# fusioninfer/fusioninfer

Hardware: AMD Instinct MI355X
Metric: goodput req/s (Qwen3-8B serving, closed-loop) (higher is better)
Workload: dtype bf16; 1 GPU; model=Qwen3-8B, global_batch=256, seq_len=1152, prompt_len=1024, gen_len=128, parallelism=dp1

## Files before the change

### fusioninfer_amd/engine/model_runner.py

```python

from __future__ import annotations

import os
from typing import Dict, List, Optional, Tuple

import numpy as np
import torch

from fusioninfer_amd.config import EngineConfig
from fusioninfer_amd.engine.block_manager import BlockManager
from fusioninfer_amd.engine.metadata import AttnMetadata
from fusioninfer_amd.engine.sequence import Sequence
from fusioninfer_amd.models.model import CausalLM
import fusioninfer_amd.ops as ops_mod

_DECODE_BUCKETS = [1, 2, 4, 8, 16, 24, 32, 48, 64, 96, 128, 160, 192, 224, 256, 320, 384, 448, 512]


class ModelRunner:
    def __init__(self, cfg: EngineConfig, device: str):
        self.cfg = cfg
        self.device = torch.device(device)
        self.is_cuda = self.device.type == "cuda"
        mc = cfg.model
# ... 149 lines not shown
            "lora_names": [s.lora_name for s in seqs],
        }

    def _lora_route(self, prefill_payload, decode_payload, np_=0):
        if self.lora_registry is None:
            return None
        spans: List[Tuple[int, int, str]] = []
        total = 0
        if prefill_payload is not None:
            cu = prefill_payload["cu"]
            total = cu[-1]
            for i, name in enumerate(prefill_payload.get("lora_names") or []):
                if name:
                    spans.append((cu[i], cu[i + 1], name))
        if decode_payload is not None:
            total = np_ + len(decode_payload["lens"])
            for i, name in enumerate(decode_payload.get("lora_names") or []):
                if name:
                    spans.append((np_ + i, np_ + i + 1, name))
        if not spans:
            return None
        reg = self.lora_registry
        adapters = {}
        for _, _, name in spans:
            if name not in adapters:
                adapters[name] = reg.get(name)
        if self.lora_slots is not None and len(adapters) <= reg.max_loras:
            slot = {name: reg.slot_of(name) for name in adapters}
            if all(s is not None for s in slot.values()):
                ids = np.full(total, -1, dtype=np.int32)
                for a, b, name in spans:
                    ids[a:b] = slot[name]
                self.num_lora_slot_steps += 1
                return "slots", ids
        groups: Dict[str, List[int]] = {}
        for a, b, name in spans:
            groups.setdefault(name, []).extend(range(a, b))
        self.num_lora_loop_steps += 1
        return "loop", [(adapters[n], rows) for n, rows in groups.items()]

    def _lora_batch(self, prefill_payload, decode_payload, np_=0):
        route = self._lora_route(prefill_payload, decode_payload, np_)
        if route is None:
            return None
        from fusioninfer_amd.lora import LoRABatch

        kind, data = route
        if kind == "slots":
            return LoRABatch(
                slot_ids=torch.from_numpy(data).to(self.device),
                slots=self.lora_slots,
            )
        return self._lora_batch_from_groups(data)

    def _lora_batch_from_groups(self, groups):
        from fusioninfer_amd.lora import LoRABatch

        return LoRABatch(
            [
                (
                    adapter,
                    torch.tensor(rows, dtype=torch.long, device=self.device),
                )
                for adapter, rows in groups
            ]
        )

    def run_prefill(self, payload) -> torch.Tensor:
        import fusioninfer_amd.distributed.parallel_state as ps

        if ps.pp_world_size() > 1:
            subs = self._split_prefill_payload(payload)
            if len(subs) > 1:
                return self._run_prefill_pp_pipelined(subs)
        ids, meta, logits_idx = self._prefill_inputs(payload)
        with torch.no_grad():
            return self._forward_and_logits(ids, meta, logits_idx)

    def _prefill_inputs(self, payload):
        dev = self.device
        cu = payload["cu"]
        tile_rows = ops_mod.prefill_tile_rows(payload["new_lens"])
        tile_seq, tile_row0 = ops_mod.build_prefill_tiles(
            payload["new_lens"], device=dev, rows=tile_rows
        )
        meta = AttnMetadata(
            num_prefill_tokens=cu[-1],
            num_decode_tokens=0,
            positions=torch.tensor(
                payload["positions"], dtype=torch.int32, device=dev
            ),
            slot_mapping=torch.tensor(
                payload["slots"], dtype=torch.int32, device=dev
            ),
            cu_seqlens=torch.tensor(cu, dtype=torch.int32, device=dev),
            tile_seq=tile_seq,
            tile_rows=tile_rows,
            tile_row0=tile_row0,
            prefill_block_tables=torch.tensor(
                payload["bt"], dtype=torch.int32, device=dev
            ),
            prefill_seq_lens_k=torch.tensor(
                payload["total_lens"], dtype=torch.int32, device=dev
            ),
        )
        meta.lora = self._lora_batch(payload, None)
        ids = torch.tensor(payload["ids"], dtype=torch.long, device=dev)
        if payload.get("logits_rows") is not None:
            logits_idx = torch.tensor(
                payload["logits_rows"], dtype=torch.long, device=dev
            )
        else:
            sample = payload.get("sample") or [True] * (len(cu) - 1)
            logits_idx = torch.tensor(
                [c - 1 for c, smp in zip(cu[1:], sample) if smp],
                dtype=torch.long,
                device=dev,
            )
        return ids, meta, logits_idx

    def _split_prefill_payload(self, payload, min_mb_tokens: int = 256):
        import fusioninfer_amd.distributed.parallel_state as ps

        cu = payload["cu"]
        n_seqs = len(cu) - 1
        M = min(ps.pp_world_size(), n_seqs, cu[-1] // min_mb_tokens)
        if M < 2:
            return [payload]
        target = cu[-1] / M
        bounds = [0]
        for i in range(1, M):
            want = i * target
            j = bounds[-1] + 1
            while j < n_seqs - (M - 1 - i) and cu[j + 1] <= want:
                j += 1
            bounds.append(j)
        bounds.append(n_seqs)
        rows = payload.get("logits_rows")
        subs = []
        for a, b in zip(bounds, bounds[1:]):
            lo, hi = cu[a], cu[b]
            sp = {
                "kind": "prefill",
                "ids": payload["ids"][lo:hi],
                "positions": payload["positions"][lo:hi],
                "slots": payload["slots"][lo:hi],
                "cu": [c - lo for c in cu[a: b + 1]],
                "new_lens": payload["new_lens"][a:b],
                "total_lens": payload["total_lens"][a:b],
                "bt": payload["bt"][a:b],
                "sample": payload["sample"][a:b],
                "lora_names": (payload.get("lora_names") or [None] * n_seqs)[a:b],
            }
            if rows is not None:
                sp["logits_rows"] = [r - lo for r in rows if lo <= r < hi]
            subs.append(sp)
        return subs

    def _run_prefill_pp_pipelined(self, subs) -> torch.Tensor:
        import fusioninfer_amd.distributed.parallel_state as ps

        V = self.cfg.model.vocab_size
        H = self.cfg.model.hidden_size
        dt = torch.bfloat16
        dev = self.device
        last = ps.pp_world_size() - 1
        inputs = [self._prefill_inputs(sp) for sp in subs]
# ... 112 lines not shown
        payload["kind"] = "mixed"
        d = (
            self.build_decode_payload(decode_seqs, bm)
            if decode_seqs
            else {"ids": [], "positions": [], "slots": [], "lens": [], "bt": []}
        )
        payload["decode"] = d
        return payload

    def build_spec_payload(
        self,
        prefill_seqs: List[Sequence],
        chunks: List[int],
        decode_seqs: List[Sequence],
        drafts: List[List[int]],
        bm: BlockManager,
    ):
        input_ids: List[int] = []
        positions: List[int] = []
        slots: List[int] = []
        cu = [0]
        new_lens: List[int] = []
        total_lens: List[int] = []
        sample: List[bool] = []
        logits_rows: List[int] = []
        bs = bm.block_size
        all_seqs = list(prefill_seqs) + list(decode_seqs)

        def _extend(seq, toks, C):
            chunk = len(toks)
            input_ids.extend(toks)
            positions.extend(range(C, C + chunk))
            pos = np.arange(C, C + chunk)
            blocks = np.asarray(seq.block_ids, dtype=np.int64)
            slots.extend((blocks[pos // bs] * bs + pos % bs).tolist())
            cu.append(cu[-1] + chunk)
            new_lens.append(chunk)
            total_lens.append(C + chunk)

        for seq, chunk in zip(prefill_seqs, chunks):
            C = seq.num_computed_tokens or seq.num_cached_tokens
            _extend(seq, seq.all_token_ids[C: C + chunk], C)
            done = C + chunk >= seq.num_prompt_tokens
            sample.append(done)
            if done:
                logits_rows.append(cu[-1] - 1)
        for seq, draft in zip(decode_seqs, drafts):
            row0 = cu[-1]
            _extend(seq, [seq.all_token_ids[-1]] + list(draft),
                    seq.num_tokens - 1)
            sample.append(True)
            logits_rows.extend(range(row0, cu[-1]))
        max_blocks = max(len(s.block_ids) for s in all_seqs)
        bt = [
            s.block_ids + [0] * (max_blocks - len(s.block_ids))
            for s in all_seqs
        ]
        return {
            "kind": "prefill",
            "ids": input_ids,
            "positions": positions,
            "slots": slots,
            "cu": cu,
            "new_lens": new_lens,
            "total_lens": total_lens,
            "bt": bt,
            "sample": sample,
            "logits_rows": logits_rows,
            "lora_names": [s.lora_name for s in all_seqs],
        }

    def run_batch(self, payload) -> torch.Tensor:
        d = payload["decode"]
        if not payload["ids"]:
            return self.run_decode(d)
        if not d["ids"]:
            return self.run_prefill(payload)
        dev = self.device
        cu = payload["cu"]
        np_ = cu[-1]
        nd = len(d["ids"])
        tile_rows = ops_mod.prefill_tile_rows(payload["new_lens"])
        tile_seq, tile_row0 = ops_mod.build_prefill_tiles(
            payload["new_lens"], device=dev, rows=tile_rows
        )
        max_blocks = max(len(b) for b in d["bt"])
        dbt_np = np.zeros((nd, max_blocks), dtype=np.int32)
        for i, ids in enumerate(d["bt"]):
            dbt_np[i, : len(ids)] = ids
        dbt = torch.from_numpy(dbt_np)
        meta = AttnMetadata(
            num_prefill_tokens=np_,
            num_decode_tokens=nd,
            positions=torch.tensor(
                payload["positions"] + d["positions"],
                dtype=torch.int32, device=dev,
            ),
            slot_mapping=torch.tensor(
                payload["slots"] + d["slots"], dtype=torch.int32, device=dev
            ),
            cu_seqlens=torch.tensor(cu, dtype=torch.int32, device=dev),
            tile_seq=tile_seq,
            tile_rows=tile_rows,
            tile_row0=tile_row0,
            prefill_block_tables=torch.tensor(
                payload["bt"], dtype=torch.int32, device=dev
            ),
            prefill_seq_lens_k=torch.tensor(
                payload["total_lens"], dtype=torch.int32, device=dev
            ),
            block_tables=dbt.to(dev),
            seq_lens=torch.tensor(d["lens"], dtype=torch.int32, device=dev),
        )
        meta.lora = self._lora_batch(payload, d, np_=np_)
        ids = torch.tensor(
            payload["ids"] + d["ids"], dtype=torch.long, device=dev
        )
        if payload.get("logits_rows") is not None:
            logits_idx = torch.tensor(
                payload["logits_rows"], dtype=torch.long, device=dev
            )
        else:
            pf_idx = [
                c - 1 for c, smp in zip(cu[1:], payload["sample"]) if smp
            ]
            logits_idx = torch.tensor(
                pf_idx + list(range(np_, np_ + nd)), dtype=torch.long,
                device=dev,
            )
        with torch.no_grad():
            return self._forward_and_logits(ids, meta, logits_idx)

    def _alloc_static(self, max_bs: int) -> None:
        dev = self.device
        self._static = {
            "ids": torch.zeros(max_bs, dtype=torch.long, device=dev),
            "positions": torch.zeros(max_bs, dtype=torch.int32, device=dev),
            "slots": torch.full((max_bs,), -1, dtype=torch.int32, device=dev),
            "block_tables": torch.zeros(
                (max_bs, self.max_blocks_per_seq), dtype=torch.int32, device=dev
            ),
            "seq_lens": torch.ones(max_bs, dtype=torch.int32, device=dev),
        }
        if self.lora_slots is not None:
            self._static["lora_slots"] = torch.full(
                (max_bs,), -1, dtype=torch.int32, device=dev
            )

    def _decode_forward(self, bs: int, lora=None) -> torch.Tensor:
        s = self._static
        meta = AttnMetadata(
            num_prefill_tokens=0,
            num_decode_tokens=bs,
            lora=lora,
            positions=s["positions"][:bs],
            slot_mapping=s["slots"][:bs],
            block_tables=s["block_tables"][:bs],
            seq_lens=s["seq_lens"][:bs],
        )
        return self._forward_and_logits(
            s["ids"][:bs], meta,
            torch.arange(bs, dtype=torch.long, device=self.device),
        )

    def capture_decode_graphs(self) -> None:
        import fusioninfer_amd.distributed.parallel_state as ps

# ... 139 lines not shown
```

### fusioninfer_amd/ops/__init__.py

```python

from __future__ import annotations

import math
from typing import Optional

import torch

from fusioninfer_amd.ops import reference as ref

_C = None
_C_IMPORT_ERROR: Optional[BaseException] = None
try:
    import importlib

    _C = importlib.import_module("fusioninfer_amd.ops._C")
except Exception as e:
    _C_IMPORT_ERROR = e


def has_native() -> bool:
    return _C is not None


def _require_native():
# ... 170 lines not shown
        _require_native()
        n = int(block_ids.numel())
        staging = torch.empty(
            (2, n, *k_cache.shape[1:]), dtype=k_cache.dtype, device=k_cache.device
        )
        _C.gather_kv_blocks(staging, k_cache, v_cache, block_ids)
        return staging
    return ref.gather_kv_blocks(k_cache, v_cache, block_ids.long())


def scatter_kv_blocks(staging, k_cache, v_cache, block_ids):
    if k_cache.is_cuda:
        _require_native()
        _C.scatter_kv_blocks(staging, k_cache, v_cache, block_ids)
        return
    ref.scatter_kv_blocks(staging, k_cache, v_cache, block_ids.long())



DECODE_PARTITION_TOKENS = 512


def _check_attn_out(out: torch.Tensor, q: torch.Tensor) -> None:
    if (out.shape != q.shape or out.dtype != q.dtype
            or out.device != q.device or not out.is_contiguous()):
        raise ValueError(
            f"out must be a contiguous {tuple(q.shape)} {q.dtype} tensor on "
            f"{q.device}, got {tuple(out.shape)} {out.dtype} strides "
            f"{out.stride()} on {out.device}")


def paged_attention_decode(
    q: torch.Tensor,
    k_cache: torch.Tensor,
    v_cache: torch.Tensor,
    block_tables: torch.Tensor,
    seq_lens: torch.Tensor,
    scale: Optional[float] = None,
    out: Optional[torch.Tensor] = None,
) -> torch.Tensor:
    if scale is None:
        scale = 1.0 / math.sqrt(q.shape[-1])
    if out is not None:
        _check_attn_out(out, q)
    if q.is_cuda:
        _require_native()
        S, Hq, D = q.shape
        if out is None:
            out = torch.empty(q.shape, dtype=q.dtype, device=q.device)
        max_tokens = int(block_tables.shape[1]) * int(k_cache.shape[2])
        num_parts = max(
            (max_tokens + DECODE_PARTITION_TOKENS - 1) // DECODE_PARTITION_TOKENS,
            1,
        )
        ml_ws = acc_ws = None
        if num_parts > 1:
            ml_ws = torch.empty(
                (S, Hq, num_parts, 2), dtype=torch.float32, device=q.device
            )
            acc_ws = torch.empty(
                (S, Hq, num_parts, D), dtype=torch.float32, device=q.device
            )
        _C.paged_attention_decode(
            out, q, k_cache, v_cache, block_tables, seq_lens,
            ml_ws, acc_ws, num_parts, scale,
        )
        return out
    res = ref.paged_attention_decode(q, k_cache, v_cache, block_tables, seq_lens, scale)
    return res if out is None else out.copy_(res)


import os as _os

PREFILL_TILE_ROWS = (4 if _os.environ.get("FI_PF_NW", "8").startswith("4")
                     else 8) * 32


def prefill_tile_rows(seq_lens) -> int:
    if seq_lens and max(seq_lens) >= 4096:
        return 128
    return PREFILL_TILE_ROWS


def build_prefill_tiles(seq_lens, device=None, rows=None):
    rows = rows or PREFILL_TILE_ROWS
    tile_seq, tile_row0 = [], []
    for s, L in enumerate(seq_lens):
        for r0 in range(0, L, rows):
            tile_seq.append(s)
            tile_row0.append(r0)
    return (
        torch.tensor(tile_seq, dtype=torch.int32, device=device),
        torch.tensor(tile_row0, dtype=torch.int32, device=device),
    )


def prefill_attention(
    q: torch.Tensor,
    k: torch.Tensor,
    v: torch.Tensor,
    cu_seqlens: torch.Tensor,
    scale: Optional[float] = None,
    tile_seq: Optional[torch.Tensor] = None,
    tile_row0: Optional[torch.Tensor] = None,
    tile_rows: Optional[int] = None,
) -> torch.Tensor:
    if scale is None:
        scale = 1.0 / math.sqrt(q.shape[-1])
    if q.is_cuda:
        _require_native()
        if tile_seq is None:
            lens = (cu_seqlens[1:] - cu_seqlens[:-1]).tolist()
            tile_rows = tile_rows or prefill_tile_rows(lens)
            tile_seq, tile_row0 = build_prefill_tiles(
                lens, device=q.device, rows=tile_rows
            )
        out = torch.empty(q.shape, dtype=q.dtype, device=q.device)
        _C.prefill_attention(out, q, k, v, tile_seq, tile_row0, cu_seqlens,
                             scale, tile_rows or PREFILL_TILE_ROWS)
        return out
    return ref.prefill_attention(q, k, v, cu_seqlens, scale, causal=True)


def prefill_attention_paged(
    q: torch.Tensor,
    k_cache: torch.Tensor,
    v_cache: torch.Tensor,
    block_tables: torch.Tensor,
    cu_seqlens_q: torch.Tensor,
    seq_lens_k: torch.Tensor,
    scale: Optional[float] = None,
    tile_seq: Optional[torch.Tensor] = None,
    tile_row0: Optional[torch.Tensor] = None,
    tile_rows: Optional[int] = None,
    out: Optional[torch.Tensor] = None,
) -> torch.Tensor:
    if scale is None:
        scale = 1.0 / math.sqrt(q.shape[-1])
    if out is not None:
        _check_attn_out(out, q)
    if q.is_cuda:
        _require_native()
        if tile_seq is None:
            lens = (cu_seqlens_q[1:] - cu_seqlens_q[:-1]).tolist()
            tile_rows = tile_rows or prefill_tile_rows(lens)
            tile_seq, tile_row0 = build_prefill_tiles(
                lens, device=q.device, rows=tile_rows
            )
        if out is None:
            out = torch.empty(q.shape, dtype=q.dtype, device=q.device)
        _C.prefill_attention_paged(
            out, q, k_cache, v_cache, tile_seq, tile_row0, cu_seqlens_q,
            block_tables, seq_lens_k, scale,
            tile_rows or PREFILL_TILE_ROWS,
        )
        return out
    res = ref.prefill_attention_paged(
        q, k_cache, v_cache, block_tables, cu_seqlens_q, seq_lens_k, scale
    )
    return res if out is None else out.copy_(res)



def pack_moe_weights(w: torch.Tensor) -> torch.Tensor:
    E, K, N = w.shape
    assert K % 32 == 0 and N % 16 == 0, (K, N)
    return (
        w.view(E, K // 32, 4, 8, N // 16, 16)
        .permute(0, 1, 4, 2, 5, 3)
        .reshape(E, K // 32, N // 16, 64, 8)
        .contiguous()
    )


def moe_gemm(out, a, b_packed, sorted_ids, expert_ids, n_valid,
             block_m: int, gate_up: bool):
    if out.is_cuda:
        _require_native()
        _C.moe_gemm(out, a, b_packed, sorted_ids, expert_ids, n_valid,
                    block_m, gate_up)
        return out
    return ref.moe_gemm(out, a, b_packed, sorted_ids, expert_ids, n_valid,
                        block_m, gate_up)


def moe_gemm_fp8(out, a, a_scales, b_packed, b_scales, sorted_ids,
                 expert_ids, n_valid, block_m: int, gate_up: bool):
    if out.is_cuda:
        _require_native()
        _C.moe_gemm_fp8(out, a, a_scales, b_packed, b_scales, sorted_ids,
                        expert_ids, n_valid, block_m, gate_up)
        return out
    return ref.moe_gemm_fp8(out, a, a_scales, b_packed, b_scales,
                            sorted_ids, expert_ids, n_valid, block_m,
                            gate_up)


def moe_align(topi: torch.Tensor, e_start: int, e_end: int, block_m: int):
    _require_native()
    T, k = topi.shape
    n = T * k
    E_local = e_end - e_start
    PM = ((n + block_m - 1) // block_m + E_local) * block_m
    dev = topi.device
    sorted_ids = torch.empty(PM, dtype=torch.int32, device=dev)
    expert_ids = torch.empty(PM // block_m, dtype=torch.int32, device=dev)
    n_valid = torch.empty(1, dtype=torch.int32, device=dev)
    pos = torch.empty(n, dtype=torch.int32, device=dev)
    _C.moe_align(topi.reshape(-1).int().contiguous(), sorted_ids,
                 expert_ids, n_valid, pos, k, e_start, e_end, block_m)
    return sorted_ids, expert_ids, n_valid, pos, PM


def moe_router_topk(logits: torch.Tensor, k: int, renorm: bool):
    _require_native()
    T, E = logits.shape
    topv = torch.empty(T, k, dtype=torch.float32, device=logits.device)
    topi = torch.empty(T, k, dtype=torch.int32, device=logits.device)
    _C.moe_router_topk(logits.contiguous(), topv, topi, k, renorm)
    return topv, topi


def moe_combine(out, y, pos, w):
    if out.is_cuda:
        _require_native()
        _C.moe_combine(out, y, pos, w)
        return out
    return ref.moe_combine(out, y, pos, w)



LORA_MAX_RANK = 128


def lora_shapes_supported(K: int, N: int, R: int) -> bool:
    return (K % 64 == 0 and N % 16 == 0 and R % 16 == 0
            and 16 <= R <= LORA_MAX_RANK)
# ... 217 lines not shown
```

### fusioninfer_amd/ops/csrc/ops.hip

```cpp

#include <torch/extension.h>

#include <c10/hip/HIPStream.h>
#include <hip/hip_runtime.h>

#include "common.h"

namespace fi {

template <bool FUSED_ADD, bool FP8_OUT>
void launch_rms_norm(void*, float*, const u16*, u16*, const u16*, float, int,
                     int, hipStream_t);
void launch_silu_and_mul(u16*, const u16*, int64_t, int, hipStream_t);
template <bool SILU_MUL>
void launch_row_quant_fp8(unsigned char*, float*, const u16*, int, int,
                          hipStream_t);
void launch_rope_qk_norm(u16*, u16*, int64_t, int64_t, const u16*, const u16*,
                         const float*, const int*, int, int, int, int, float,
                         hipStream_t);
void launch_reshape_and_cache(const u16*, const u16*, void*, void*,
                              const int*, int64_t, int64_t, int, int, int,
                              int, bool, float, float, hipStream_t);
void launch_rope_qk_norm_cache(u16*, const u16*, const u16*, int64_t, int64_t,
                               int64_t, const u16*, const u16*, const float*,
                               const int*, void*, void*, const int*, int, int,
                               int, int, float, bool, float, float,
                               hipStream_t);
template <bool GATHER>
void launch_kv_block_copy(u16*, u16*, u16*, const int*, int, int64_t,
                          hipStream_t);
void launch_paged_attn_decode(u16*, float*, float*, const u16*, const void*,
                              const void*, const int*, const int*, int,
                              int64_t, int, int, int, int, int, float, bool,
                              hipStream_t);
void launch_prefill_attn(u16*, const u16*, const void*, const void*,
                         const int*, const int*, const int*, const int*,
                         const int*, int, int, int64_t, int64_t, int64_t, int,
                         int, int, float, bool, int, hipStream_t);
void launch_moe_gemm(u16*, const u16*, const u16*, const int*, const int*,
                     const int*, int, int, int, int, bool, hipStream_t);
void launch_moe_gemm_fp8(u16*, const unsigned char*, const float*,
                         const unsigned char*, const float*, const int*,
                         const int*, const int*, int, int, int, int, bool,
                         hipStream_t);
void launch_moe_align(const int*, int*, int*, int*, int*, int, int, int,
                      int, int, int, hipStream_t);
void launch_moe_router_topk(const float*, float*, int*, int, int, int,
                            bool, hipStream_t);
void launch_moe_combine(u16*, const u16*, const int*, const float*, int, int,
                        int, hipStream_t);
void launch_lora_apply(u16*, u16*, const u16*, const int*, const u16*,
                       const u16*, const float*, int, int, int, int, int,
                       hipStream_t);
void launch_sample_tokens(int64_t*, const float*, const float*, const int*,
                          const float*, const float*, const int64_t*, int,
                          int, hipStream_t);
void launch_token_logprobs(float*, int*, float*, const float*, const int64_t*,
                           const int*, int, int, int, hipStream_t);
void launch_apply_penalties(float*, const int*, const int*, const float*, int,
                            int, int, hipStream_t);
void launch_penalty_counts_add(int*, const int*, const int64_t*, int, int,
                               int, hipStream_t);

}

namespace {

using fi::u16;

#define CHECK_BF16_CUDA(t)                                     \
  TORCH_CHECK((t).is_cuda(), #t " must be on GPU");            \
  TORCH_CHECK((t).scalar_type() == at::kBFloat16, #t " must be bf16")

u16* bf16_ptr(at::Tensor& t) { return reinterpret_cast<u16*>(t.data_ptr()); }
const u16* bf16_cptr(const at::Tensor& t) {
  return reinterpret_cast<const u16*>(t.data_ptr());
}

hipStream_t current_stream() {
  return c10::hip::getCurrentHIPStream().stream();
}

bool cache_is_fp8(const at::Tensor& t) {
  TORCH_CHECK(
      t.scalar_type() == at::kBFloat16 || t.scalar_type() == at::kFloat8_e4m3fn,
      "kv cache must be bf16 or float8_e4m3fn");
  return t.scalar_type() == at::kFloat8_e4m3fn;
}

void rms_norm(at::Tensor out, at::Tensor input, at::Tensor weight, double eps) {
  CHECK_BF16_CUDA(out);
  CHECK_BF16_CUDA(input);
  TORCH_CHECK(input.is_contiguous() && out.is_contiguous());
  const int hidden = input.size(-1);
  const int tokens = input.numel() / hidden;
  fi::launch_rms_norm<false, false>(bf16_ptr(out), nullptr, bf16_cptr(input),
                                    nullptr, bf16_cptr(weight),
                                    static_cast<float>(eps), tokens, hidden,
                                    current_stream());
}

void fused_add_rms_norm(at::Tensor input, at::Tensor residual,
                        at::Tensor weight, double eps) {
  CHECK_BF16_CUDA(input);
  CHECK_BF16_CUDA(residual);
  TORCH_CHECK(input.is_contiguous() && residual.is_contiguous());
  const int hidden = input.size(-1);
  const int tokens = input.numel() / hidden;
  fi::launch_rms_norm<true, false>(bf16_ptr(input), nullptr, bf16_cptr(input),
                                   bf16_ptr(residual), bf16_cptr(weight),
                                   static_cast<float>(eps), tokens, hidden,
                                   current_stream());
}

#define CHECK_FP8_OUT(o, s)                                                  \
  TORCH_CHECK((o).scalar_type() == at::kFloat8_e4m3fn && (o).is_cuda() &&    \
              (o).is_contiguous());                                          \
  TORCH_CHECK((s).scalar_type() == at::kFloat && (s).is_cuda())

void rms_norm_fp8(at::Tensor out, at::Tensor out_scales, at::Tensor input,
                  at::Tensor weight, double eps) {
// ... 156 lines not shown
  const u16* qw = weight_ptr(q_weight);
  const u16* kw = weight_ptr(k_weight);
  fi::launch_rope_qk_norm_cache(
      bf16_ptr(q), bf16_cptr(k), bf16_cptr(v), q.stride(0), k.stride(0),
      v.stride(0), qw, kw, cos_sin.data_ptr<float>(),
      positions.data_ptr<int>(), k_cache.data_ptr(), v_cache.data_ptr(),
      slot_mapping.data_ptr<int>(), static_cast<int>(tokens),
      static_cast<int>(num_q_heads), static_cast<int>(num_kv_heads),
      static_cast<int>(head_dim), static_cast<float>(eps), fp8,
      static_cast<float>(k_inv_scale), static_cast<float>(v_inv_scale),
      current_stream());
}

void gather_kv_blocks(at::Tensor staging, at::Tensor k_cache,
                      at::Tensor v_cache, at::Tensor block_ids) {
  TORCH_CHECK(staging.is_cuda() &&
              staging.scalar_type() == k_cache.scalar_type());
  TORCH_CHECK(block_ids.scalar_type() == at::kInt);
  const int n = block_ids.size(0);
  const int64_t block_elems = k_cache.size(1) * k_cache.size(2) *
      k_cache.size(3) * k_cache.element_size() / 2;
  fi::launch_kv_block_copy<true>(
      static_cast<fi::u16*>(staging.data_ptr()),
      static_cast<fi::u16*>(k_cache.data_ptr()),
      static_cast<fi::u16*>(v_cache.data_ptr()), block_ids.data_ptr<int>(), n,
      block_elems, current_stream());
}

void scatter_kv_blocks(at::Tensor staging, at::Tensor k_cache,
                       at::Tensor v_cache, at::Tensor block_ids) {
  TORCH_CHECK(staging.is_cuda() &&
              staging.scalar_type() == k_cache.scalar_type());
  TORCH_CHECK(block_ids.scalar_type() == at::kInt);
  const int n = block_ids.size(0);
  const int64_t block_elems = k_cache.size(1) * k_cache.size(2) *
      k_cache.size(3) * k_cache.element_size() / 2;
  fi::launch_kv_block_copy<false>(
      static_cast<fi::u16*>(staging.data_ptr()),
      static_cast<fi::u16*>(k_cache.data_ptr()),
      static_cast<fi::u16*>(v_cache.data_ptr()), block_ids.data_ptr<int>(), n,
      block_elems, current_stream());
}

void paged_attention_decode(at::Tensor out, at::Tensor q, at::Tensor k_cache,
                            at::Tensor v_cache, at::Tensor block_tables,
                            at::Tensor seq_lens,
                            c10::optional<at::Tensor> ml_ws,
                            c10::optional<at::Tensor> acc_ws,
                            int64_t num_parts, double scale) {
  CHECK_BF16_CUDA(out);
  CHECK_BF16_CUDA(q);
  const bool fp8 = cache_is_fp8(k_cache);
  TORCH_CHECK(block_tables.scalar_type() == at::kInt &&
              block_tables.is_contiguous());
  TORCH_CHECK(seq_lens.scalar_type() == at::kInt);
  TORCH_CHECK(q.dim() == 3);
  const int num_seqs = q.size(0);
  const int num_heads = q.size(1);
  const int head_dim = q.size(2);
  const int num_kv_heads = k_cache.size(1);
  TORCH_CHECK(k_cache.size(2) == 16, "cache block_size must be 16");
  TORCH_CHECK(q.stride(2) == 1 && q.stride(1) == head_dim);
  TORCH_CHECK(out.is_contiguous() && out.sizes() == q.sizes(),
              "out must be a contiguous [S, Hq, D] tensor");
  float* ml = nullptr;
  float* acc = nullptr;
  if (num_parts > 1) {
    TORCH_CHECK(ml_ws && acc_ws, "workspace required when num_parts > 1");
    ml = ml_ws->data_ptr<float>();
    acc = acc_ws->data_ptr<float>();
  }
  fi::launch_paged_attn_decode(
      bf16_ptr(out), ml, acc, bf16_cptr(q), k_cache.data_ptr(),
      v_cache.data_ptr(), block_tables.data_ptr<int>(),
      seq_lens.data_ptr<int>(), num_seqs, q.stride(0), block_tables.size(1),
      num_kv_heads, head_dim, num_heads / num_kv_heads,
      static_cast<int>(num_parts), static_cast<float>(scale), fp8,
      current_stream());
}

void prefill_attention(at::Tensor out, at::Tensor q, at::Tensor k,
                       at::Tensor v, at::Tensor tile_seq, at::Tensor tile_row0,
                       at::Tensor cu_seqlens, double scale,
                       int64_t tile_rows) {
  TORCH_CHECK(tile_rows == 128 || tile_rows == 256,
              "tile_rows must be 128 or 256");
  CHECK_BF16_CUDA(out);
  CHECK_BF16_CUDA(q);
  TORCH_CHECK(tile_seq.scalar_type() == at::kInt &&
              tile_row0.scalar_type() == at::kInt &&
              cu_seqlens.scalar_type() == at::kInt);
  TORCH_CHECK(q.dim() == 3 && k.dim() == 3 && v.dim() == 3);
  const int num_q_heads = q.size(1);
  const int head_dim = q.size(2);
  const int num_kv_heads = k.size(1);
  TORCH_CHECK(q.stride(2) == 1 && q.stride(1) == head_dim);
  TORCH_CHECK(k.stride(2) == 1 && k.stride(1) == head_dim);
  TORCH_CHECK(v.stride(2) == 1 && v.stride(1) == head_dim);
  fi::launch_prefill_attn(
      bf16_ptr(out), bf16_cptr(q), bf16_cptr(k), bf16_cptr(v),
      tile_seq.data_ptr<int>(), tile_row0.data_ptr<int>(),
      cu_seqlens.data_ptr<int>(), nullptr, nullptr, 0, tile_seq.size(0),
      q.stride(0), k.stride(0), v.stride(0), num_q_heads, num_kv_heads,
      head_dim, static_cast<float>(scale), false,
      static_cast<int>(tile_rows / 32), current_stream());
}

void prefill_attention_paged(at::Tensor out, at::Tensor q, at::Tensor k_cache,
                             at::Tensor v_cache, at::Tensor tile_seq,
                             at::Tensor tile_row0, at::Tensor cu_seqlens,
                             at::Tensor block_tables, at::Tensor seq_lens_k,
                             double scale, int64_t tile_rows) {
  TORCH_CHECK(tile_rows == 128 || tile_rows == 256,
              "tile_rows must be 128 or 256");
  CHECK_BF16_CUDA(out);
  CHECK_BF16_CUDA(q);
  const bool fp8 = cache_is_fp8(k_cache);
  TORCH_CHECK(tile_seq.scalar_type() == at::kInt &&
              tile_row0.scalar_type() == at::kInt &&
              cu_seqlens.scalar_type() == at::kInt &&
              block_tables.scalar_type() == at::kInt &&
              seq_lens_k.scalar_type() == at::kInt);
  TORCH_CHECK(block_tables.is_contiguous());
  TORCH_CHECK(q.dim() == 3);
  const int num_q_heads = q.size(1);
  const int head_dim = q.size(2);
  const int num_kv_heads = k_cache.size(1);
  TORCH_CHECK(k_cache.size(2) == 16, "cache block_size must be 16");
  TORCH_CHECK(q.stride(2) == 1 && q.stride(1) == head_dim);
  TORCH_CHECK(out.is_contiguous() && out.sizes() == q.sizes(),
              "out must be a contiguous [T, Hq, D] tensor");
  fi::launch_prefill_attn(
      bf16_ptr(out), bf16_cptr(q), k_cache.data_ptr(), v_cache.data_ptr(),
      tile_seq.data_ptr<int>(), tile_row0.data_ptr<int>(),
      cu_seqlens.data_ptr<int>(), block_tables.data_ptr<int>(),
      seq_lens_k.data_ptr<int>(), block_tables.size(1), tile_seq.size(0),
      q.stride(0), 0, 0, num_q_heads, num_kv_heads, head_dim,
      static_cast<float>(scale), fp8,
      static_cast<int>(tile_rows / 32), current_stream());
}

struct MoeGemmDims {
  int K, N, max_mtiles;
};

MoeGemmDims check_moe_gemm(const at::Tensor& out, const at::Tensor& a,
                           const at::Tensor& b_packed,
                           const at::Tensor& sorted_ids,
                           const at::Tensor& expert_ids,
                           const at::Tensor& n_valid, int64_t block_m,
                           bool gate_up) {
  TORCH_CHECK(sorted_ids.scalar_type() == at::kInt &&
              expert_ids.scalar_type() == at::kInt &&
              n_valid.scalar_type() == at::kInt);
  TORCH_CHECK(block_m == 16 || block_m == 128, "block_m must be 16 or 128");
  const int K = a.size(1);
  const int N = out.size(1);
  const int PM = out.size(0);
  TORCH_CHECK(PM % block_m == 0, "padded rows must be block_m-aligned");
  TORCH_CHECK(K % 32 == 0, "K must be a multiple of 32");
  TORCH_CHECK(
      N % (block_m == 16 ? 64 : (gate_up ? 64 : 128)) == 0,
      "N tile misalignment");
  TORCH_CHECK(b_packed.dim() == 5 && b_packed.size(1) == K / 32 &&
              b_packed.size(2) == (gate_up ? 2 * N : N) / 16 &&
              b_packed.size(3) == 64 && b_packed.size(4) == 8,
              "b_packed layout mismatch");
  TORCH_CHECK(expert_ids.size(0) >= PM / block_m);
  if (gate_up) TORCH_CHECK(sorted_ids.size(0) >= PM);
  return {K, N, static_cast<int>(PM / block_m)};
}

void moe_gemm(at::Tensor out, at::Tensor a, at::Tensor b_packed,
              at::Tensor sorted_ids, at::Tensor expert_ids,
              at::Tensor n_valid, int64_t block_m, bool gate_up) {
  CHECK_BF16_CUDA(out);
  CHECK_BF16_CUDA(a);
  CHECK_BF16_CUDA(b_packed);
  TORCH_CHECK(out.is_contiguous() && a.is_contiguous() &&
              b_packed.is_contiguous());
  const MoeGemmDims d = check_moe_gemm(out, a, b_packed, sorted_ids,
                                       expert_ids, n_valid, block_m, gate_up);
  fi::launch_moe_gemm(bf16_ptr(out), bf16_cptr(a),
                      bf16_cptr(b_packed), sorted_ids.data_ptr<int>(),
                      expert_ids.data_ptr<int>(), n_valid.data_ptr<int>(),
                      d.max_mtiles, d.K, d.N, static_cast<int>(block_m),
                      gate_up, current_stream());
}

void moe_gemm_fp8(at::Tensor out, at::Tensor a, at::Tensor a_scales,
                  at::Tensor b_packed, at::Tensor b_scales,
                  at::Tensor sorted_ids, at::Tensor expert_ids,
                  at::Tensor n_valid, int64_t block_m, bool gate_up) {
  CHECK_BF16_CUDA(out);
  TORCH_CHECK(a.scalar_type() == at::kFloat8_e4m3fn && a.is_cuda() &&
              a.is_contiguous());
  TORCH_CHECK(b_packed.scalar_type() == at::kFloat8_e4m3fn &&
              b_packed.is_contiguous());
  TORCH_CHECK(a_scales.scalar_type() == at::kFloat &&
              b_scales.scalar_type() == at::kFloat &&
              b_scales.is_contiguous());
  const MoeGemmDims d = check_moe_gemm(out, a, b_packed, sorted_ids,
                                       expert_ids, n_valid, block_m, gate_up);
  TORCH_CHECK(b_scales.numel() ==
              b_packed.size(0) * (gate_up ? 2 * d.N : d.N));
  fi::launch_moe_gemm_fp8(
      bf16_ptr(out), static_cast<const unsigned char*>(a.data_ptr()),
      a_scales.data_ptr<float>(),
      static_cast<const unsigned char*>(b_packed.data_ptr()),
      b_scales.data_ptr<float>(), sorted_ids.data_ptr<int>(),
      expert_ids.data_ptr<int>(), n_valid.data_ptr<int>(), d.max_mtiles,
      d.K, d.N, static_cast<int>(block_m), gate_up, current_stream());
}

void moe_combine(at::Tensor out, at::Tensor y, at::Tensor pos, at::Tensor w) {
  CHECK_BF16_CUDA(out);
  CHECK_BF16_CUDA(y);
  TORCH_CHECK(out.is_contiguous() && y.is_contiguous());
  TORCH_CHECK(pos.scalar_type() == at::kInt && pos.is_contiguous());
  TORCH_CHECK(w.scalar_type() == at::kFloat && w.is_contiguous());
  const int T = out.size(0);
  const int H = out.size(1);
// ... 255 lines not shown
```

### fusioninfer_amd/ops/csrc/prefill_attention.hip

```cpp

#include "common.h"

#include <type_traits>

namespace fi {

typedef __attribute__((ext_vector_type(8))) short short8;
typedef __attribute__((ext_vector_type(16))) float floatx16;

constexpr int kWaves = 8;
constexpr int kQPerWave = 32;
constexpr int kQBlock = kWaves * kQPerWave;
constexpr int kKVTile = 64;
constexpr float kPNegInf = -1e30f;
constexpr float kDeferThr = 11.5416f;

template <int ROWB>
FI_DEV int swz(int row, int byte_in_row) {
  constexpr int kMask = (ROWB / 16 > 16 ? 16 : ROWB / 16) - 1;
  return row * ROWB + (byte_in_row ^ ((row & kMask) << 4));
}

FI_DEV constexpr int crow(int r, int hi1) {
  return (r & 3) + 8 * (r >> 2) + 4 * hi1;
}

FI_DEV u32 pack_bf16x2(float lo, float hi) {
  return static_cast<u32>(f32_to_bf16(lo)) |
         (static_cast<u32>(f32_to_bf16(hi)) << 16);
}

template <int D, bool PAGED, bool FP8, int WPS = 2, int NW = kWaves>
__global__ __launch_bounds__(NW * kWaveSize, WPS) void prefill_attn_kernel(
    u16* __restrict__ out,
    const u16* __restrict__ q,
    const void* __restrict__ k_p,
    const void* __restrict__ v_p,
    const int* __restrict__ tile_seq,
    const int* __restrict__ tile_row0,
    const int* __restrict__ cu_seqlens,
    const int* __restrict__ block_tables,
    const int* __restrict__ seq_lens_k,
    const int max_blocks,
    const int64_t q_stride, const int64_t k_stride, const int64_t v_stride,
    const int num_q_heads, const int num_kv_heads, const float scale) {
  using CT = typename std::conditional<FP8, unsigned char, u16>::type;
  const CT* k = static_cast<const CT*>(k_p);
  const CT* v = static_cast<const CT*>(v_p);
  constexpr int KF = D / 16;
  constexpr int CB = D / 32;
  constexpr int kKRowB = D * 2;
  constexpr int kVTRowB = 128;

  const int head = blockIdx.y;
  const int kv_head = head / (num_q_heads / num_kv_heads);
  const int tid = threadIdx.x;
  const int wave = tid / kWaveSize;
  const int lane = tid % kWaveSize;
  const int col = lane & 31;
  const int hi1 = lane >> 5;

  const int seq = tile_seq[blockIdx.x];
  const int seq_start = cu_seqlens[seq];
  const int seq_len = cu_seqlens[seq + 1] - seq_start;
  const int k_len = PAGED ? seq_lens_k[seq] : seq_len;
  const int ctx_start = k_len - seq_len;
  const int wg_row0 = tile_row0[blockIdx.x];
  const int row0 = wg_row0 + wave * kQPerWave;
  const bool active = row0 < seq_len;
  const int* bt_row = PAGED
      ? block_tables + static_cast<int64_t>(seq) * max_blocks : nullptr;
  auto kv_off = [&](int r, int64_t dense_stride) -> int64_t {
    if (PAGED) {
      const int blk = bt_row[r >> 4];
      return ((static_cast<int64_t>(blk) * num_kv_heads + kv_head) * 16 +
              (r & 15)) * D;
    }
    return (seq_start + r) * dense_stride + static_cast<int64_t>(kv_head) * D;
  };

  __shared__ u16 smem[3 * kKVTile * D + 2 * D * (kVTRowB / 2)];
  auto k_lds = [&](int i) -> u16* { return smem + i * (kKVTile * D); };
  u16* vt_lds0 = smem + 3 * kKVTile * D;
  u16* vt_lds1 = vt_lds0 + D * (kVTRowB / 2);

  short8 b_q[KF];
  if (active) {
    const int qr = min(row0 + col, seq_len - 1);
    const u16* qrow = q + (seq_start + qr) * q_stride +
                      static_cast<int64_t>(head) * D;
    const float qs = scale * 1.4426950408889634f;
#pragma unroll
    for (int f = 0; f < KF; ++f) {
      short8 raw = *reinterpret_cast<const short8*>(qrow + f * 16 + hi1 * 8);
      bf16x8 h = __builtin_bit_cast(bf16x8, raw);
#pragma unroll
      for (int j = 0; j < 8; ++j)
        h.h[j] = f32_to_bf16(bf16_to_f32(h.h[j]) * qs);
      b_q[f] = __builtin_bit_cast(short8, h);
    }
  }

  float m_row = kPNegInf, l_row = 0.f;
  floatx16 o_acc[CB];
#pragma unroll
  for (int cb = 0; cb < CB; ++cb)
#pragma unroll
    for (int r = 0; r < 16; ++r) o_acc[cb][r] = 0.f;

  const int wg_q_max = ctx_start + min(wg_row0 + NW * kQPerWave, seq_len) - 1;
  const int num_kv_tiles = wg_q_max / kKVTile + 1;
  const int my_q_max = ctx_start + min(row0 + kQPerWave, seq_len) - 1;

  constexpr int kKTileBytes = kKVTile * kKRowB;
  constexpr int kGldsPerWave = kKTileBytes / (NW * kWaveSize * 16);
  auto stage_k_glds = [&](int t, u16* kbuf) {
    const int kv0 = t * kKVTile;
#pragma unroll
    for (int i = 0; i < kGldsPerWave; ++i) {
      const int base_off = wave * (kKTileBytes / NW) + i * (kWaveSize * 16);
      const int X = base_off + lane * 16;
      const int row = X / kKRowB;
      const int sbyte = X % kKRowB;
      constexpr int kMask = (kKRowB / 16 > 16 ? 16 : kKRowB / 16) - 1;
      const int byte = sbyte ^ ((row & kMask) << 4);
      const int src_row = min(kv0 + row, k_len - 1);
      const CT* gsrc = k + kv_off(src_row, k_stride) + byte / sizeof(u16);
      __builtin_amdgcn_global_load_lds(
          (const __attribute__((address_space(1))) void*)gsrc,
          (__attribute__((address_space(3))) void*)(
              reinterpret_cast<char*>(kbuf) + base_off),
          16, 0, 0);
    }
  };
  constexpr int kChunks = D / 16;
  constexpr int VITER = ceil_div(kChunks, NW);
  const int v_kv = tid % kKVTile;
  const int v_c0 = tid / kKVTile;
  auto cvt_fp8x16 = [](uint4 raw, bf16x8& lo, bf16x8& hi) {
    const u32 w[4] = {raw.x, raw.y, raw.z, raw.w};
    float f[16];
#pragma unroll
    for (int i = 0; i < 4; ++i) unpack_fp8x4(w[i], &f[i * 4]);
#pragma unroll
    for (int j = 0; j < 8; ++j) {
      lo.h[j] = f32_to_bf16(f[j]);
      hi.h[j] = f32_to_bf16(f[8 + j]);
    }
  };
  bf16x8 vreg0[VITER], vreg1[VITER];
// ... 181 lines not shown
#pragma unroll
          for (int cb = 0; cb < CB; ++cb) o_acc[cb][r] *= a_r;
        }
      }
    }

    if (compute) {
      const char* vbase = reinterpret_cast<const char*>(vt_cur);
      short8 a_p[4];
#pragma unroll
      for (int b = 0; b < 2; ++b)
#pragma unroll
        for (int c = 0; c < 2; ++c) {
          const int base = 8 * c;
          const u32 u1 = pack_bf16x2(s_acc[b][base + 0], s_acc[b][base + 1]);
          const u32 u2 = pack_bf16x2(s_acc[b][base + 2], s_acc[b][base + 3]);
          const u32 v1 = pack_bf16x2(s_acc[b][base + 4], s_acc[b][base + 5]);
          const u32 v2 = pack_bf16x2(s_acc[b][base + 6], s_acc[b][base + 7]);
          const auto s1 = __builtin_amdgcn_permlane32_swap(
              static_cast<int>(u1), static_cast<int>(v1), false, false);
          const auto s2 = __builtin_amdgcn_permlane32_swap(
              static_cast<int>(u2), static_cast<int>(v2), false, false);
          typedef __attribute__((ext_vector_type(4))) unsigned int u32x4;
          u32x4 w;
          w.x = static_cast<u32>(s1[0]);
          w.y = static_cast<u32>(s2[0]);
          w.z = static_cast<u32>(s1[1]);
          w.w = static_cast<u32>(s2[1]);
          a_p[2 * b + c] = __builtin_bit_cast(short8, w);
        }

      __builtin_amdgcn_s_setprio(1);
#pragma unroll
      for (int kc = 0; kc < 4; ++kc) {
#pragma unroll
        for (int cb = 0; cb < CB; ++cb) {
          const short8 b_v =
              *reinterpret_cast<const short8*>(vbase + v_off[kc][cb]);
          o_acc[cb] = __builtin_amdgcn_mfma_f32_32x32x16_bf16(
              a_p[kc], b_v, o_acc[cb], 0, 0, 0);
        }
      }
      __builtin_amdgcn_s_setprio(0);
    }
    if (FP8) {
      if (t + 1 < num_kv_tiles) {
        kwrite_fp8(kbuf_next);
        vwrite(vt_next);
        if (t + 2 < num_kv_tiles) {
          kload_fp8(t + 2);
          vload(t + 2);
        }
      }
      __syncthreads();
    } else {
      vwrite(vt_next);
      vload(t + 2);
      tile_barrier();
    }
  }

  if (active) {
    const float inv_own = (l_row > 0.f) ? 1.f / l_row : 0.f;
#pragma unroll
    for (int r = 0; r < 16; ++r) {
      const int qr = row0 + crow(r, hi1);
      if (qr >= seq_len) continue;
      const float inv = __shfl(inv_own, crow(r, hi1), 64);
      u16* orow = out + (static_cast<int64_t>(seq_start + qr) * num_q_heads +
                         head) * D;
#pragma unroll
      for (int cb = 0; cb < CB; ++cb)
        orow[cb * 32 + col] = f32_to_bf16(o_acc[cb][r] * inv);
    }
  }
}

void launch_prefill_attn(u16* out, const u16* q, const void* k, const void* v,
                         const int* tile_seq, const int* tile_row0,
                         const int* cu_seqlens, const int* block_tables,
                         const int* seq_lens_k, int max_blocks, int ntiles,
                         int64_t q_stride, int64_t k_stride, int64_t v_stride,
                         int num_q_heads, int num_kv_heads, int head_dim,
                         float scale, bool fp8, int nw, hipStream_t stream) {
  const bool paged = block_tables != nullptr;
  dim3 grid(ntiles, num_q_heads), block(nw * kWaveSize);
#define FI_PF_LAUNCH(DD, PP, F8)                                              \
  do {                                                                        \
    if (nw == 4)                                                              \
      hipLaunchKernelGGL((prefill_attn_kernel<DD, PP, F8, 2, 4>), grid,       \
                         block, 0, stream, out, q, k, v, tile_seq,            \
                         tile_row0, cu_seqlens, block_tables, seq_lens_k,     \
                         max_blocks, q_stride, k_stride, v_stride,            \
                         num_q_heads, num_kv_heads, scale);                   \
    else                                                                      \
      hipLaunchKernelGGL((prefill_attn_kernel<DD, PP, F8, 2, 8>), grid,       \
                         block, 0, stream, out, q, k, v, tile_seq,            \
                         tile_row0, cu_seqlens, block_tables, seq_lens_k,     \
                         max_blocks, q_stride, k_stride, v_stride,            \
                         num_q_heads, num_kv_heads, scale);                   \
  } while (0)
  if (fp8 && !paged) abort();
  if (head_dim == 128) {
    if (paged) {
      if (fp8) FI_PF_LAUNCH(128, true, true);
      else FI_PF_LAUNCH(128, true, false);
    } else {
      FI_PF_LAUNCH(128, false, false);
    }
  } else if (head_dim == 64) {
    if (paged) {
      if (fp8) FI_PF_LAUNCH(64, true, true);
      else FI_PF_LAUNCH(64, true, false);
    } else {
      FI_PF_LAUNCH(64, false, false);
    }
  } else {
    abort();
  }
#undef FI_PF_LAUNCH
}

}
```

Baseline: 49.04 req/s.

## Schedule prefill attention tiles heaviest-first with heads adjacent in a 1D grid

Prefill attention tiles are now sorted by estimated causal KV cost, so the longest tiles launch first and the tail of the grid is made of short tiles. The grid is also flattened to 1D with all query heads of a tile adjacent, so workgroups sharing the same K/V run together and can reuse it in cache. Both behaviours sit behind an environment flag that defaults to on. The cost is some extra host-side sorting per batch and a divide in the kernel prologue.

```diff
diff --git a/fusioninfer_amd/engine/model_runner.py b/fusioninfer_amd/engine/model_runner.py
--- a/fusioninfer_amd/engine/model_runner.py
+++ b/fusioninfer_amd/engine/model_runner.py
@@ -255,7 +255,11 @@
         cu = payload["cu"]
         tile_rows = ops_mod.prefill_tile_rows(payload["new_lens"])
         tile_seq, tile_row0 = ops_mod.build_prefill_tiles(
-            payload["new_lens"], device=dev, rows=tile_rows
+            payload["new_lens"], device=dev, rows=tile_rows,
+            ctx_starts=[
+                t - n
+                for t, n in zip(payload["total_lens"], payload["new_lens"])
+            ],
         )
         meta = AttnMetadata(
             num_prefill_tokens=cu[-1],
@@ -534,7 +538,11 @@
         nd = len(d["ids"])
         tile_rows = ops_mod.prefill_tile_rows(payload["new_lens"])
         tile_seq, tile_row0 = ops_mod.build_prefill_tiles(
-            payload["new_lens"], device=dev, rows=tile_rows
+            payload["new_lens"], device=dev, rows=tile_rows,
+            ctx_starts=[
+                t - n
+                for t, n in zip(payload["total_lens"], payload["new_lens"])
+            ],
         )
         max_blocks = max(len(b) for b in d["bt"])
         dbt_np = np.zeros((nd, max_blocks), dtype=np.int32)
diff --git a/fusioninfer_amd/ops/__init__.py b/fusioninfer_amd/ops/__init__.py
--- a/fusioninfer_amd/ops/__init__.py
+++ b/fusioninfer_amd/ops/__init__.py
@@ -276,13 +276,27 @@
     return PREFILL_TILE_ROWS
 
 
-def build_prefill_tiles(seq_lens, device=None, rows=None):
+PF_TILE_ORDER = _os.environ.get("FI_PF_TILE_ORDER", "1") != "0"
+
+PREFILL_KV_TILE = 64
+
+
+def build_prefill_tiles(seq_lens, device=None, rows=None, ctx_starts=None,
+                        heaviest_first=None):
     rows = rows or PREFILL_TILE_ROWS
-    tile_seq, tile_row0 = [], []
-    for s, L in enumerate(seq_lens):
+    if heaviest_first is None:
+        heaviest_first = PF_TILE_ORDER
+    if ctx_starts is None:
+        ctx_starts = [0] * len(seq_lens)
+    tiles = []
+    for s, (L, c) in enumerate(zip(seq_lens, ctx_starts)):
         for r0 in range(0, L, rows):
-            tile_seq.append(s)
-            tile_row0.append(r0)
+            cost = -(-(c + min(r0 + rows, L)) // PREFILL_KV_TILE)
+            tiles.append((-cost, s, r0))
+    if heaviest_first:
+        tiles.sort()
+    tile_seq = [t[1] for t in tiles]
+    tile_row0 = [t[2] for t in tiles]
     return (
         torch.tensor(tile_seq, dtype=torch.int32, device=device),
         torch.tensor(tile_row0, dtype=torch.int32, device=device),
@@ -311,7 +325,8 @@
             )
         out = torch.empty(q.shape, dtype=q.dtype, device=q.device)
         _C.prefill_attention(out, q, k, v, tile_seq, tile_row0, cu_seqlens,
-                             scale, tile_rows or PREFILL_TILE_ROWS)
+                             scale, tile_rows or PREFILL_TILE_ROWS,
+                             PF_TILE_ORDER)
         return out
     return ref.prefill_attention(q, k, v, cu_seqlens, scale, causal=True)
 
@@ -337,16 +352,17 @@
         _require_native()
         if tile_seq is None:
             lens = (cu_seqlens_q[1:] - cu_seqlens_q[:-1]).tolist()
+            ctx = [k_len - n for k_len, n in zip(seq_lens_k.tolist(), lens)]
             tile_rows = tile_rows or prefill_tile_rows(lens)
             tile_seq, tile_row0 = build_prefill_tiles(
-                lens, device=q.device, rows=tile_rows
+                lens, device=q.device, rows=tile_rows, ctx_starts=ctx
             )
         if out is None:
             out = torch.empty(q.shape, dtype=q.dtype, device=q.device)
         _C.prefill_attention_paged(
             out, q, k_cache, v_cache, tile_seq, tile_row0, cu_seqlens_q,
             block_tables, seq_lens_k, scale,
-            tile_rows or PREFILL_TILE_ROWS,
+            tile_rows or PREFILL_TILE_ROWS, PF_TILE_ORDER,
         )
         return out
     res = ref.prefill_attention_paged(
diff --git a/fusioninfer_amd/ops/csrc/ops.hip b/fusioninfer_amd/ops/csrc/ops.hip
--- a/fusioninfer_amd/ops/csrc/ops.hip
+++ b/fusioninfer_amd/ops/csrc/ops.hip
@@ -36,7 +36,7 @@
 void launch_prefill_attn(u16*, const u16*, const void*, const void*,
                          const int*, const int*, const int*, const int*,
                          const int*, int, int, int64_t, int64_t, int64_t, int,
-                         int, int, float, bool, int, hipStream_t);
+                         int, int, float, bool, int, bool, hipStream_t);
 void launch_moe_gemm(u16*, const u16*, const u16*, const int*, const int*,
                      const int*, int, int, int, int, bool, hipStream_t);
 void launch_moe_gemm_fp8(u16*, const unsigned char*, const float*,
@@ -359,7 +359,7 @@
 void prefill_attention(at::Tensor out, at::Tensor q, at::Tensor k,
                        at::Tensor v, at::Tensor tile_seq, at::Tensor tile_row0,
                        at::Tensor cu_seqlens, double scale,
-                       int64_t tile_rows) {
+                       int64_t tile_rows, bool heads_adjacent) {
   TORCH_CHECK(tile_rows == 128 || tile_rows == 256,
               "tile_rows must be 128 or 256");
   CHECK_BF16_CUDA(out);
@@ -374,20 +374,23 @@
   TORCH_CHECK(q.stride(2) == 1 && q.stride(1) == head_dim);
   TORCH_CHECK(k.stride(2) == 1 && k.stride(1) == head_dim);
   TORCH_CHECK(v.stride(2) == 1 && v.stride(1) == head_dim);
+  TORCH_CHECK(tile_seq.size(0) * q.size(1) < (int64_t{1} << 31),
+              "too many (tile, head) workgroups for one grid");
   fi::launch_prefill_attn(
       bf16_ptr(out), bf16_cptr(q), bf16_cptr(k), bf16_cptr(v),
       tile_seq.data_ptr<int>(), tile_row0.data_ptr<int>(),
       cu_seqlens.data_ptr<int>(), nullptr, nullptr, 0, tile_seq.size(0),
       q.stride(0), k.stride(0), v.stride(0), num_q_heads, num_kv_heads,
       head_dim, static_cast<float>(scale), false,
-      static_cast<int>(tile_rows / 32), current_stream());
+      static_cast<int>(tile_rows / 32), heads_adjacent, current_stream());
 }
 
 void prefill_attention_paged(at::Tensor out, at::Tensor q, at::Tensor k_cache,
                              at::Tensor v_cache, at::Tensor tile_seq,
                              at::Tensor tile_row0, at::Tensor cu_seqlens,
                              at::Tensor block_tables, at::Tensor seq_lens_k,
-                             double scale, int64_t tile_rows) {
+                             double scale, int64_t tile_rows,
+                             bool heads_adjacent) {
   TORCH_CHECK(tile_rows == 128 || tile_rows == 256,
               "tile_rows must be 128 or 256");
   CHECK_BF16_CUDA(out);
@@ -407,6 +410,8 @@
   TORCH_CHECK(q.stride(2) == 1 && q.stride(1) == head_dim);
   TORCH_CHECK(out.is_contiguous() && out.sizes() == q.sizes(),
               "out must be a contiguous [T, Hq, D] tensor");
+  TORCH_CHECK(tile_seq.size(0) * q.size(1) < (int64_t{1} << 31),
+              "too many (tile, head) workgroups for one grid");
   fi::launch_prefill_attn(
       bf16_ptr(out), bf16_cptr(q), k_cache.data_ptr(), v_cache.data_ptr(),
       tile_seq.data_ptr<int>(), tile_row0.data_ptr<int>(),
@@ -414,7 +419,7 @@
       seq_lens_k.data_ptr<int>(), block_tables.size(1), tile_seq.size(0),
       q.stride(0), 0, 0, num_q_heads, num_kv_heads, head_dim,
       static_cast<float>(scale), fp8,
-      static_cast<int>(tile_rows / 32), current_stream());
+      static_cast<int>(tile_rows / 32), heads_adjacent, current_stream());
 }
 
 struct MoeGemmDims {
diff --git a/fusioninfer_amd/ops/csrc/prefill_attention.hip b/fusioninfer_amd/ops/csrc/prefill_attention.hip
--- a/fusioninfer_amd/ops/csrc/prefill_attention.hip
+++ b/fusioninfer_amd/ops/csrc/prefill_attention.hip
@@ -43,7 +43,8 @@
     const int* __restrict__ seq_lens_k,
     const int max_blocks,
     const int64_t q_stride, const int64_t k_stride, const int64_t v_stride,
-    const int num_q_heads, const int num_kv_heads, const float scale) {
+    const int num_q_heads, const int num_kv_heads, const float scale,
+    const int heads_adjacent) {
   using CT = typename std::conditional<FP8, unsigned char, u16>::type;
   const CT* k = static_cast<const CT*>(k_p);
   const CT* v = static_cast<const CT*>(v_p);
@@ -52,7 +53,12 @@
   constexpr int kKRowB = D * 2;
   constexpr int kVTRowB = 128;
 
-  const int head = blockIdx.y;
+  int head = blockIdx.y, tile = blockIdx.x;
+  if (heads_adjacent) {
+    const int id = blockIdx.x;
+    tile = __builtin_amdgcn_readfirstlane(id / num_q_heads);
+    head = id - tile * num_q_heads;
+  }
   const int kv_head = head / (num_q_heads / num_kv_heads);
   const int tid = threadIdx.x;
   const int wave = tid / kWaveSize;
@@ -60,12 +66,12 @@
   const int col = lane & 31;
   const int hi1 = lane >> 5;
 
-  const int seq = tile_seq[blockIdx.x];
+  const int seq = tile_seq[tile];
   const int seq_start = cu_seqlens[seq];
   const int seq_len = cu_seqlens[seq + 1] - seq_start;
   const int k_len = PAGED ? seq_lens_k[seq] : seq_len;
   const int ctx_start = k_len - seq_len;
-  const int wg_row0 = tile_row0[blockIdx.x];
+  const int wg_row0 = tile_row0[tile];
   const int row0 = wg_row0 + wave * kQPerWave;
   const bool active = row0 < seq_len;
   const int* bt_row = PAGED
@@ -413,9 +419,14 @@
                          const int* seq_lens_k, int max_blocks, int ntiles,
                          int64_t q_stride, int64_t k_stride, int64_t v_stride,
                          int num_q_heads, int num_kv_heads, int head_dim,
-                         float scale, bool fp8, int nw, hipStream_t stream) {
+                         float scale, bool fp8, int nw, bool heads_adjacent,
+                         hipStream_t stream) {
   const bool paged = block_tables != nullptr;
-  dim3 grid(ntiles, num_q_heads), block(nw * kWaveSize);
+  const dim3 grid = heads_adjacent
+      ? dim3(static_cast<unsigned>(ntiles) * num_q_heads)
+      : dim3(ntiles, num_q_heads);
+  const dim3 block(nw * kWaveSize);
+  const int adj = heads_adjacent ? 1 : 0;
 #define FI_PF_LAUNCH(DD, PP, F8)                                              \
   do {                                                                        \
     if (nw == 4)                                                              \
@@ -423,13 +434,13 @@
                          block, 0, stream, out, q, k, v, tile_seq,            \
                          tile_row0, cu_seqlens, block_tables, seq_lens_k,     \
                          max_blocks, q_stride, k_stride, v_stride,            \
-                         num_q_heads, num_kv_heads, scale);                   \
+                         num_q_heads, num_kv_heads, scale, adj);              \
     else                                                                      \
       hipLaunchKernelGGL((prefill_attn_kernel<DD, PP, F8, 2, 8>), grid,       \
                          block, 0, stream, out, q, k, v, tile_seq,            \
                          tile_row0, cu_seqlens, block_tables, seq_lens_k,     \
                          max_blocks, q_stride, k_stride, v_stride,            \
-                         num_q_heads, num_kv_heads, scale);                   \
+                         num_q_heads, num_kv_heads, scale, adj);              \
   } while (0)
   if (fp8 && !paged) abort();
   if (head_dim == 128) {
```

New measurement: 49.96 req/s, median of 6. 1.9% higher.
